# cristicbz/rust-doom

Measured on NVIDIA H100. Metric: frames/sec at 1920x1080 (palette-index bit-exact), higher is better.
Workload: dtype u8

## Files before the change

### rust-doom_b200/csrc/b2d_kernels.cu

```cuda
#include "b2d_kernels.cuh"

namespace b2d {

namespace {

constexpr unsigned kFull = 0xFFFFFFFFu;

constexpr int kMaskWords = 128;
constexpr int kStackDepth = 128;

constexpr uint32_t kVisBit = 1u << 25, kSolidBit = 1u << 24;
__device__ __forceinline__ uint32_t pack_range(int lo, int hi, uint32_t bits) {
    return (uint32_t)lo | ((uint32_t)hi << 12) | bits;
}
__device__ __forceinline__ int range_lo(uint32_t r) { return (int)(r & 0xFFFu); }
__device__ __forceinline__ int range_hi(uint32_t r) { return (int)((r >> 12) & 0xFFFu); }

__device__ __forceinline__ uint32_t word_bits(int w, int lo, int hi) {
    int a = max(lo, w * 32), b = min(hi, w * 32 + 31);
    if (a > b) return 0u;
    uint32_t m = 0xFFFFFFFFu >> (31 - (b - w * 32));
    return m & (0xFFFFFFFFu << (a - w * 32));
}

__device__ __forceinline__ bool range_open(const uint32_t *mask, int lane, int lo, int hi, int passes) {
    bool open = false;
#pragma unroll
    for (int k = 0; k < kMaskWords / 32; k++) {
        if (k >= passes) break;
        int w = lane + 32 * k;
        uint32_t bits = word_bits(w, lo, hi);
        if (bits & ~mask[w]) open = true;
    }
    return __any_sync(kFull, open);
}

__device__ __forceinline__ bool lane_range_open(const uint32_t *mask, int lo, int hi) {
    for (int w = lo >> 5; w <= (hi >> 5); w++)
        if (word_bits(w, lo, hi) & ~mask[w]) return true;
    return false;
}

__device__ __forceinline__ void mark_solid(uint32_t *mask, int lane, int lo, int hi, int passes) {
#pragma unroll
    for (int k = 0; k < kMaskWords / 32; k++) {
        if (k >= passes) break;
        int w = lane + 32 * k;
        uint32_t bits = word_bits(w, lo, hi);
        if (bits) mask[w] |= bits;
    }
}

__host__ __device__ inline size_t align16(size_t v) { return (v + 15) & ~(size_t)15; }

struct WalkSmem {
    size_t off_tx, off_tz, off_segr, off_boxr, off_node, off_ssec, off_sprr, off_sprz, off_mask, off_stack, off_list, total;
};
__host__ __device__ inline WalkSmem walk_layout(int nverts, int nsegs, int nnodes, int nss, int nsprites) {
    WalkSmem L;
    size_t o = 0;
    L.off_tx = o; o = align16(o + 4 * (size_t)nverts);
    L.off_tz = o; o = align16(o + 4 * (size_t)nverts);
    L.off_segr = o; o = align16(o + 4 * (size_t)nsegs);
    L.off_boxr = o; o = align16(o + 8 * (size_t)nnodes);
    L.off_node = o; o = align16(o + 32 * (size_t)nnodes);
    L.off_ssec = o; o = align16(o + 16 * (size_t)nss);
    L.off_sprr = o; o = align16(o + 4 * (size_t)nsprites);
    L.off_sprz = o; o = align16(o + 4 * (size_t)nsprites);
    L.off_mask = o; o = align16(o + 4 * kMaskWords);
    L.off_stack = o; o = align16(o + 4 * kStackDepth);
    L.off_list = o; o = align16(o + 2 * ((size_t)nsegs + (size_t)nsprites));
    L.total = o;
    return L;
}

__device__ __forceinline__ uint32_t smem_addr(const void *p) { return (uint32_t)__cvta_generic_to_shared(p); }
__device__ __forceinline__ void mbar_init(uint64_t *bar, uint32_t arrivals) {
    asm volatile("mbarrier.init.shared::cta.b64 [%0], %1;" ::"r"(smem_addr(bar)), "r"(arrivals));
    asm volatile("fence.mbarrier_init.release.cluster;" ::: "memory");
}
__device__ __forceinline__ void bulk_copy_g2s(void *dst, const void *src, uint32_t bytes, uint64_t *bar) {
    asm volatile("mbarrier.arrive.expect_tx.shared::cta.b64 _, [%0], %1;" ::"r"(smem_addr(bar)), "r"(bytes) : "memory");
    asm volatile("cp.async.bulk.shared::cluster.global.mbarrier::complete_tx::bytes [%0], [%1], %2, [%3];"
                 ::"r"(smem_addr(dst)), "l"(src), "r"(bytes), "r"(smem_addr(bar)) : "memory");
}
__device__ __forceinline__ bool mbar_wait(uint64_t *bar, uint32_t parity) {
    for (int spin = 0; spin < (1 << 24); spin++) {
        uint32_t done;
        asm volatile("{\n\t.reg .pred p;\n\tmbarrier.try_wait.parity.shared::cta.b64 p, [%1], %2;\n\tselp.u32 %0, 1, 0, p;\n\t}"
                     : "=r"(done) : "r"(smem_addr(bar)), "r"(parity) : "memory");
        if (done) return true;
    }
    return false;
}

__global__ void __launch_bounds__(128, 7)
b2d_walk_kernel(const __grid_constant__ DeviceScene sc, const __grid_constant__ View vw, const Pose *__restrict__ poses, int n,
                FrameConst *__restrict__ frames, SegFrame *__restrict__ work, int stride) {
    extern __shared__ __align__(16) uint8_t smem[];
    const int lane = threadIdx.x & 31, warp = threadIdx.x >> 5;
    const int tid = threadIdx.x, nthr = blockDim.x;
    const WalkSmem L = walk_layout(sc.nverts, sc.nsegs, sc.nnodes, sc.nss, sc.nsprites);
    uint8_t *base = smem;
    __shared__ int s_count, s_status;
    __shared__ __align__(8) uint64_t s_bar;
    int32_t *tx = reinterpret_cast<int32_t *>(base + L.off_tx);
    int32_t *tz = reinterpret_cast<int32_t *>(base + L.off_tz);
    uint32_t *segr = reinterpret_cast<uint32_t *>(base + L.off_segr);
    uint32_t *boxr = reinterpret_cast<uint32_t *>(base + L.off_boxr);
    int4 *node_s = reinterpret_cast<int4 *>(base + L.off_node);
    int4 *ssec_s = reinterpret_cast<int4 *>(base + L.off_ssec);
    uint32_t *sprr = reinterpret_cast<uint32_t *>(base + L.off_sprr);
    int32_t *sprz = reinterpret_cast<int32_t *>(base + L.off_sprz);
    uint32_t *mask = reinterpret_cast<uint32_t *>(base + L.off_mask);
    uint32_t *stack = reinterpret_cast<uint32_t *>(base + L.off_stack);
    uint16_t *list = reinterpret_cast<uint16_t *>(base + L.off_list);

    const uint32_t static_bytes = 32u * (uint32_t)sc.nnodes + 16u * (uint32_t)sc.nss;
    bool static_pending = false;
    if (static_bytes) {
        if (tid == 0) mbar_init(&s_bar, 1);
        __syncthreads();
        if (tid == 0) bulk_copy_g2s(node_s, sc.walk_static, static_bytes, &s_bar);
        static_pending = true;
    }
    for (int frame = blockIdx.x; frame < n; frame += gridDim.x) {
    FrameConst fc;
    frame_setup(poses[frame], fc);

    for (int i = tid; i < sc.nverts; i += nthr) {
        int32_t vx = sc.verts[2 * i], vy = sc.verts[2 * i + 1];
        int32_t a, b;
        to_view(fc, vx, vy, a, b);
        tx[i] = a; tz[i] = b;
    }
    __syncthreads();

    for (int i = tid; i < sc.nsegs; i += nthr) {
        const SegRec &S = sc.segs[i];
        uint32_t packed = 0;
        int32_t flags = S.flags;
        if (!(flags & kSegInvalid)) {
            SegFrame sf;
            const bool closes = seg_closes(flags & kSegTwoSided, S.otop, S.obot);
            if (seg_frame_setup(vw, tx[S.v1], tz[S.v1], tx[S.v2], tz[S.v2], sf, closes))
                packed = pack_range(sf.xlo, sf.xhi, kVisBit | (seg_solid(closes, sf) ? kSolidBit : 0u));
        }
        segr[i] = packed;
    }
    for (int i = tid; i < 2 * sc.nnodes; i += nthr) {
        const NodeRec &N = sc.nodes[i >> 1];
        const int32_t *box = (i & 1) ? N.lbox : N.rbox;
        int32_t b4[4] = {box[0], box[1], box[2], box[3]};
        int lo, hi;
        boxr[i] = box_range(fc, vw, b4, lo, hi) ? pack_range(lo, hi, kVisBit) : 0u;
    }
    if (static_pending) {
        if (!mbar_wait(&s_bar, 0)) __trap();
        static_pending = false;
    }
    for (int i = tid; i < sc.nsprites; i += nthr) {
        const SpriteRec &P = sc.sprites[i];
        SpriteFrame sp;
        uint32_t packed = 0;
        sp.cz = 0;
        if (P.tex >= 0 && P.tex < sc.ntex && sprite_setup(fc, vw, P.x, P.y, (int32_t)sc.tex[P.tex].w, sp))
            packed = pack_range(sp.lo, sp.hi, kVisBit);
        sprr[i] = packed;
        sprz[i] = (int32_t)sp.cz;
    }
    for (int w = tid; w < kMaskWords; w += nthr) mask[w] = ~word_bits(w, 0, vw.W - 1);
    if (tid == 0) stack[0] = sc.root;
    __syncthreads();

    const int passes = (vw.W + 1023) / 1024;
    int sp = warp == 0 ? 1 : 0, count = 0, status = 0;
    int budget = 2 * (sc.nnodes + sc.nss) + 64;
    while (sp > 0) {
        if (--budget < 0) { status |= kStatusNoTermination; break; }
        uint32_t child = stack[--sp];
        __syncwarp();
        if (child & kLeaf) {
            uint32_t id = child & 0x7FFFFFFFu;
            if (id >= (uint32_t)sc.nss) continue;
            const int4 ssv = ssec_s[id];
            SSectorRec ss;
            ss.first_seg = ssv.x; ss.num_segs = ssv.y; ss.sector = ssv.z; ss.sprites = ssv.w;
            if (ss.sector < 0) continue;
            {
                const int sfirst = ss.sprites & 0xFFFFFF;
                int scnt = (ss.sprites >> 24) & 0xFF;
                if (sfirst + scnt > sc.nsprites) scnt = sc.nsprites > sfirst ? sc.nsprites - sfirst : 0;
                int nvis = 0;
                for (int k0 = 0; k0 < scnt; k0 += 32) {
                    const int k = k0 + lane, pi = sfirst + k;
                    const uint32_t r = k < scnt ? sprr[pi] : 0u;
                    const bool vis = (r & kVisBit) && lane_range_open(mask, range_lo(r), range_hi(r));
                    int rank = 0, total = 0;
                    const int32_t myz = vis ? sprz[pi] : 0;
                    for (int j0 = 0; j0 < scnt; j0 += 32) {
                        const int j = j0 + lane, pj = sfirst + j;
                        const uint32_t rj = j < scnt ? sprr[pj] : 0u;
                        const bool vj = (rj & kVisBit) && lane_range_open(mask, range_lo(rj), range_hi(rj));
                        const int32_t zj = vj ? sprz[pj] : 0;
                        unsigned mj = __ballot_sync(kFull, vj);
                        total += __popc(mj);
                        while (mj) {
                            const int b = __ffs(mj) - 1;
                            mj &= mj - 1;
                            const int32_t zb = __shfl_sync(kFull, zj, b);
                            const int jb = j0 + b;
                            if (vis && (zb < myz || (zb == myz && jb < k))) rank++;
                        }
                    }
                    const int pos = count + rank;
                    if (vis && pos < sc.nsegs + sc.nsprites) list[pos] = (uint16_t)(sc.nsegs + pi);
                    nvis = total;
                }
                count = min(count + nvis, sc.nsegs + sc.nsprites);
                __syncwarp();
            }
            for (int k0 = 0; k0 < ss.num_segs; k0 += 32) {
                int k = k0 + lane;
                int si = ss.first_seg + k;
                uint32_t r = k < ss.num_segs ? segr[si] : 0u;
                bool vis = (r & kVisBit) && lane_range_open(mask, range_lo(r), range_hi(r));
                unsigned m = __ballot_sync(kFull, vis);
                int pos = count + __popc(m & ((1u << lane) - 1u));
                if (vis && pos < sc.nsegs + sc.nsprites) list[pos] = (uint16_t)si;
                count = min(count + __popc(m), sc.nsegs + sc.nsprites);
                unsigned sm = __ballot_sync(kFull, vis && (r & kSolidBit));
                __syncwarp();
                while (sm) {
                    int j = __ffs(sm) - 1;
                    sm &= sm - 1;
                    uint32_t rj = __shfl_sync(kFull, r, j);
                    mark_solid(mask, lane, range_lo(rj), range_hi(rj), passes);
                }
                __syncwarp();
            }
            if (!range_open(mask, lane, 0, vw.W - 1, passes)) break;
        } else {
            if (child >= (uint32_t)sc.nnodes) continue;
            const int4 nl = node_s[2 * child], nc = node_s[2 * child + 1];
            int side = node_side(fc.pose, nl.x, nl.y, nl.z, nl.w);
            uint32_t near_c = (uint32_t)(side ? nc.y : nc.x), far_c = (uint32_t)(side ? nc.x : nc.y);
            uint32_t rn = boxr[2 * child + side], rf = boxr[2 * child + (side ^ 1)];
            bool far_vis = (rf & kVisBit) && range_open(mask, lane, range_lo(rf), range_hi(rf), passes);
            bool near_vis = (rn & kVisBit) && range_open(mask, lane, range_lo(rn), range_hi(rn), passes);
            int need = (far_vis ? 1 : 0) + (near_vis ? 1 : 0);
            if (sp + need > kStackDepth) { status = kStatusStackOverflow; break; }
            if (lane == 0) {
                int p = sp;
                if (far_vis) stack[p++] = far_c;
                if (near_vis) stack[p++] = near_c;
            }
            sp += need;
            __syncwarp();
        }
    }
    __syncwarp();
    if (warp == 0 && lane == 0) {
        if (count > stride) { count = stride; status |= kStatusWorklistFull; }
        s_count = count; s_status = status;
    }
    __syncthreads();
    count = s_count; status = s_status;

    for (int k = tid; k < count; k += nthr) {
        int si = list[k];
        SegFrame sf;
        if (si >= sc.nsegs) {
            const int pi = si - sc.nsegs;
            const SpriteRec &P = sc.sprites[pi];
            SpriteFrame sp;
            sprite_setup(fc, vw, P.x, P.y, (int32_t)sc.tex[P.tex].w, sp);
            sprite_entry(pi, sp, sf);
            work[(size_t)frame * stride + k] = sf;
            continue;
        }
        const SegRec &S = sc.segs[si];
        seg_frame_setup(vw, tx[S.v1], tz[S.v1], tx[S.v2], tz[S.v2], sf, false);
        sf.seg = si;
        work[(size_t)frame * stride + k] = sf;
    }
    if (tid == 0) {
        if (status) atomicOr(sc.status_flag, status);
        fc.count = count;
        fc.status = status;
#pragma unroll
        for (int i = 0; i < 6; i++) fc.pad[i] = 0;
        frames[frame] = fc;
    }
    __syncthreads();
    }
}

__device__ __forceinline__ uint32_t lds_u32(uint32_t a) {
    uint32_t v;
    asm("ld.shared.u32 %0, [%1];" : "=r"(v) : "r"(a));
    return v;
}

struct RasterCtx {
    const DeviceScene *sc;
    uint32_t pal_s;
    uint2 *rowz;
    PlaneDir dir;
    uint8_t *fb;
    uint32_t *rgba;
    int W, H, x, lane;
    uint32_t skycol;
};

template <bool kRgba>
__device__ __forceinline__ void put_px(const RasterCtx &c, uint8_t *p8, uint32_t *p32, bool on, uint32_t v) {
    if (on) {
        if (kRgba) {
            *p8 = (uint8_t)v;
            *p32 = lds_u32(c.pal_s + 4u * v);
        } else {
            __stcs(p8, (uint8_t)v);
        }
    }
}

__host__ __device__ __forceinline__ bool tex_interleaved(const TexRec &T) { return b2d::tex_interleaved(T.h, T.texel_off); }

constexpr int kBatch = 8;

template <bool kRgba, int kW>
__device__ __forceinline__ void store_batch(const RasterCtx &c, uint8_t *p8, uint32_t *p32, const uint32_t (&v)[kBatch],
                                            int y, int ya, int yb, bool full) {
    const int Wc = kW ? kW : c.W;
    if (full) {
#pragma unroll
        for (int k = 0; k < kBatch; k++) put_px<kRgba>(c, p8 + (size_t)k * Wc, kRgba ? p32 + (size_t)k * Wc : nullptr, true, v[k]);
    } else {
        const uint32_t m = row_mask(y, ya, yb, kBatch);
#pragma unroll
        for (int k = 0; k < kBatch; k++)
            put_px<kRgba>(c, p8 + (size_t)k * Wc, kRgba ? p32 + (size_t)k * Wc : nullptr, (m >> k) & 1u, v[k]);
    }
}

template <bool kRgba, int kW>
__device__ __forceinline__ void fill_void_warp(const RasterCtx &c, int ya, int yb) {
    bool act = ya < yb;
    int y0 = __reduce_min_sync(kFull, act ? ya : 0x7FFFFFFF);
    int y1 = __reduce_max_sync(kFull, act ? yb : 0);
    if (y0 >= y1) return;
    const int Wc = kW ? kW : c.W;
    uint8_t *p8 = c.fb + (size_t)y0 * Wc;
    uint32_t *p32 = kRgba ? c.rgba + (size_t)y0 * Wc : nullptr;
#pragma unroll 1
    for (int y = y0; y < y1; y++, p8 += Wc, p32 += Wc) put_px<kRgba>(c, p8, p32, y >= ya && y < yb, 0u);
}

template <bool kRgba, int kW>
__device__ __forceinline__ void draw_sky_warp(const RasterCtx &c, int ya, int yb) {
    const DeviceScene &sc = *c.sc;
    if (sc.sky_tex < 0) { fill_void_warp<kRgba, kW>(c, ya, yb); return; }
    const TexRec T = sc.tex[sc.sky_tex];
    const bool inter = tex_interleaved(T);
    const uint8_t *px = sc.lit_texels + T.texel_off + (inter ? 4u * c.skycol : c.skycol);
    const uint32_t w4 = 4u * T.w;
    bool act = ya < yb;
    int y0 = __reduce_min_sync(kFull, act ? ya : 0x7FFFFFFF);
    int y1 = __reduce_max_sync(kFull, act ? yb : 0);
    if (y0 >= y1) return;
    const int Wc = kW ? kW : c.W;
    uint8_t *p8 = c.fb + (size_t)y0 * Wc;
    uint32_t *p32 = kRgba ? c.rgba + (size_t)y0 * Wc : nullptr;
#pragma unroll 2
    for (int y = y0; y < y1; y++, p8 += Wc, p32 += Wc) {
        const uint32_t r = sc.skyrow[y];
        put_px<kRgba>(c, p8, p32, y >= ya && y < yb, __ldg(px + (inter ? (r >> 2) * w4 + (r & 3u) : r * T.w)));
    }
}

template <bool kRgba, int kW>
__device__ __forceinline__ void draw_plane_warp(const RasterCtx &c, const FrameConst &fc, const View &vw,
                                                int ya, int yb, int32_t h, int32_t flat, int lightb,
                                                bool visible) {
    const DeviceScene &sc = *c.sc;
    if (!__any_sync(kFull, ya < yb)) return;
    if (!visible) { fill_void_warp<kRgba, kW>(c, ya, yb); return; }
    if (flat == kFlatSky) { draw_sky_warp<kRgba, kW>(c, ya, yb); return; }
    if (flat < 0 || flat >= sc.nflats) { fill_void_warp<kRgba, kW>(c, ya, yb); return; }
    const uint64_t px_hi = reinterpret_cast<uint64_t>(sc.lit_flats) & 0xFFFFFFFF00000000ull;
    const uint32_t habs = plane_habs(h, fc.pose.z);
    bool act = ya < yb;
    int y0 = __reduce_min_sync(kFull, act ? ya : 0x7FFFFFFF);
    int y1 = __reduce_max_sync(kFull, act ? yb : 0);
    const int full_lo = __reduce_max_sync(kFull, act ? ya : 0x7FFFFFFF);
    const int full_hi = __reduce_min_sync(kFull, act ? yb : 0);
    const int Wc = kW ? kW : c.W;
    uint8_t *p8 = c.fb + (size_t)y0 * Wc;
    uint32_t *p32 = kRgba ? c.rgba + (size_t)y0 * Wc : nullptr;
    const uint32_t bu = (uint32_t)fc.pose.x << 10, bv = (uint32_t)fc.pose.y << 10;
    const uint32_t ax = (uint32_t)c.dir.ax, ay = (uint32_t)c.dir.ay;
    for (int yc = y0; yc < y1; yc += 32) {
        int yy = yc + c.lane;
        if (yy < y1) {
            const PlaneRow pr = plane_row(habs, sc.yslope[yy]);
            c.rowz[c.lane] = make_uint2(pr.z8q, (sc.lit_flat_stride >> 6) * (uint32_t)light_row(lightb, pr.z8) + 64u * (uint32_t)flat);
        }
        __syncwarp();
        const int rows = min(32, y1 - yc);
        int j = 0;
        for (; j + kBatch <= rows; j += kBatch, p8 += (size_t)kBatch * Wc, p32 += (size_t)kBatch * Wc) {
            uint32_t v[kBatch];
#pragma unroll
            for (int k = 0; k < kBatch; k++) {
                const uint2 rz = c.rowz[j + k];
                v[k] = __ldg(reinterpret_cast<const uint8_t *>(px_hi | flat_offset(rz.y, bu + rz.x * ax, bv + rz.x * ay)));
            }
            const int y = yc + j;
            store_batch<kRgba, kW>(c, p8, p32, v, y, ya, yb, y >= full_lo && y + kBatch <= full_hi);
        }
        for (; j < rows; j++, p8 += Wc, p32 += Wc) {
            const uint2 rz = c.rowz[j];
            const int y = yc + j;
            put_px<kRgba>(c, p8, p32, y >= ya && y < yb,
                          __ldg(reinterpret_cast<const uint8_t *>(px_hi | flat_offset(rz.y, bu + rz.x * ax, bv + rz.x * ay))));
        }
        __syncwarp();
    }
}

template <bool kRgba, int kW, int R>
__device__ __forceinline__ void wall_fast_loop(const RasterCtx &c, const uint8_t *plq, uint32_t w4, uint32_t nq, uint32_t q,
                                               uint32_t acc, uint32_t ts29, int y0, int y1, int ya, int yb,
                                               int full_lo, int full_hi) {
    const int Wc = kW ? kW : c.W;
    uint8_t *p8 = c.fb + (size_t)y0 * Wc;
    uint32_t *p32 = kRgba ? c.rgba + (size_t)y0 * Wc : nullptr;
    asm("" : "+l"(plq));
#pragma unroll 1
    for (int y = y0; y < y1; y += R, p8 += (size_t)R * Wc, p32 += (size_t)R * Wc) {
        const uint32_t q1 = q + 1u == nq ? 0u : q + 1u;
        const uint32_t w0 = __ldg(reinterpret_cast<const uint32_t *>(plq + (size_t)q * w4));
        const uint32_t w1 = __ldg(reinterpret_cast<const uint32_t *>(plq + (size_t)q1 * w4));
        if (y >= full_lo && y + R <= full_hi) {
#pragma unroll
            for (int k = 0; k < R; k++) {
                uint32_t v = pick_byte(w0, w1, wall_sel(acc, ts29, (uint32_t)k));
                if (kRgba) v &= 0xFFu;
                put_px<kRgba>(c, p8 + (size_t)k * Wc, kRgba ? p32 + (size_t)k * Wc : nullptr, true, v);
            }
        } else {
            const uint32_t m = row_mask(y, ya, yb, R);
#pragma unroll
            for (int k = 0; k < R; k++) {
                uint32_t v = pick_byte(w0, w1, wall_sel(acc, ts29, (uint32_t)k));
                if (kRgba) v &= 0xFFu;
                put_px<kRgba>(c, p8 + (size_t)k * Wc, kRgba ? p32 + (size_t)k * Wc : nullptr, (m >> k) & 1u, v);
            }
        }
        wall_advance(acc, q, ts29, (uint32_t)R, nq);
    }
}

template <bool kRgba, int kW>
__device__ __forceinline__ void draw_wall_warp(const RasterCtx &c, const FrameConst &fc, int ya, int yb,
                                               int32_t tex, int32_t tA, int32_t hA, int32_t ucol,
                                               int32_t iscale, int row) {
    const DeviceScene &sc = *c.sc;
    if (!__any_sync(kFull, ya < yb)) return;
    if (tex < 0 || tex >= sc.ntex) { fill_void_warp<kRgba, kW>(c, ya, yb); return; }
    const TexRec T = sc.tex[tex];
    bool act = ya < yb;
    const uint32_t col = (uint32_t)floormod32(ucol, (int32_t)T.w);
    const uint8_t *pl = sc.lit_texels + (size_t)row * sc.lit_texel_stride + T.texel_off;
    const uint32_t tstep = (uint32_t)(iscale >> 4);
    int y0 = __reduce_min_sync(kFull, act ? ya : 0x7FFFFFFF);
    int y1 = __reduce_max_sync(kFull, act ? yb : 0);
    const int full_lo = __reduce_max_sync(kFull, act ? ya : 0x7FFFFFFF);
    const int full_hi = __reduce_min_sync(kFull, act ? yb : 0);
    uint32_t t = (uint32_t)wall_tbase(tA, hA, fc.pose.z, c.H, iscale) + (uint32_t)y0 * tstep;
    const int Wc = kW ? kW : c.W;
    uint8_t *p8 = c.fb + (size_t)y0 * Wc;
    uint32_t *p32 = kRgba ? c.rgba + (size_t)y0 * Wc : nullptr;
    if (tex_interleaved(T) && T.h >= 8u) {
        const uint32_t ts = act ? tstep : 0u;
        const bool f16 = __all_sync(kFull, ts <= kWallFast16);
        if (f16 || __all_sync(kFull, ts <= kWallFast8)) {
            const uint32_t tt = act ? t : 0u;
            const uint32_t r0 = wall_row((int32_t)tt, T.h, T.hmagic, T.hbias);
            const uint8_t *plq = pl + 4u * col;
            if (f16) wall_fast_loop<kRgba, kW, 16>(c, plq, 4u * T.w, T.h >> 2, r0 >> 2, wall_acc29(tt, r0), ts << 13, y0, y1, ya, yb, full_lo, full_hi);
            else wall_fast_loop<kRgba, kW, 8>(c, plq, 4u * T.w, T.h >> 2, r0 >> 2, wall_acc29(tt, r0), ts << 13, y0, y1, ya, yb, full_lo, full_hi);
            return;
        }
    }
    if (tex_interleaved(T)) {
        const uint32_t colb = 4u * col, w4 = 4u * T.w;
        for (int y = y0; y < y1; y += kBatch, p8 += (size_t)kBatch * Wc, p32 += (size_t)kBatch * Wc, t += (uint32_t)kBatch * tstep) {
            const uint32_t r0 = wall_row((int32_t)t, T.h, T.hmagic, T.hbias);
            const uint32_t acc = wall_acc(t, r0);
            const uint32_t b7 = (acc + 7u * tstep) >> 16;
            uint32_t v[kBatch];
            if (__all_sync(kFull, b7 < 8u)) {
                const uint32_t q0 = r0 >> 2, q1 = next_quad(q0, T.h);
                const uint32_t w0 = __ldg(reinterpret_cast<const uint32_t *>(pl + (q0 * w4 + colb)));
                const uint32_t w1 = __ldg(reinterpret_cast<const uint32_t *>(pl + (q1 * w4 + colb)));
#pragma unroll
                for (int k = 0; k < kBatch; k++) {
                    v[k] = pick_byte(w0, w1, (acc + (uint32_t)k * tstep) >> 16);
                    if (kRgba) v[k] &= 0xFFu;
                }
            } else {
                const uint32_t t4 = t + 4u * tstep;
                const uint32_t r4 = wall_row((int32_t)t4, T.h, T.hmagic, T.hbias);
                const uint32_t acc4 = wall_acc(t4, r4);
                if (__all_sync(kFull, ((acc + 3u * tstep) >> 16) < 8u && ((acc4 + 3u * tstep) >> 16) < 8u)) {
                    const uint32_t q0 = r0 >> 2, q4 = r4 >> 2;
                    const uint32_t a0 = __ldg(reinterpret_cast<const uint32_t *>(pl + (q0 * w4 + colb)));
                    const uint32_t a1 = __ldg(reinterpret_cast<const uint32_t *>(pl + (next_quad(q0, T.h) * w4 + colb)));
                    const uint32_t b0 = __ldg(reinterpret_cast<const uint32_t *>(pl + (q4 * w4 + colb)));
                    const uint32_t b1 = __ldg(reinterpret_cast<const uint32_t *>(pl + (next_quad(q4, T.h) * w4 + colb)));
#pragma unroll
                    for (int k = 0; k < 4; k++) {
                        v[k] = pick_byte(a0, a1, (acc + (uint32_t)k * tstep) >> 16);
                        v[k + 4] = pick_byte(b0, b1, (acc4 + (uint32_t)k * tstep) >> 16);
                        if (kRgba) { v[k] &= 0xFFu; v[k + 4] &= 0xFFu; }
                    }
                } else {
#pragma unroll
                    for (int k = 0; k < kBatch; k++) {
                        const uint32_t rk = wall_row((int32_t)(t + (uint32_t)k * tstep), T.h, T.hmagic, T.hbias);
                        v[k] = __ldg(pl + ((rk >> 2) * w4 + colb + (rk & 3u)));
                    }
                }
            }
            store_batch<kRgba, kW>(c, p8, p32, v, y, ya, yb, y >= full_lo && y + kBatch <= full_hi);
        }
    } else {
        const uint8_t *px = pl + col;
#pragma unroll 1
        for (int y = y0; y < y1; y++, p8 += Wc, p32 += Wc, t += tstep)
            put_px<kRgba>(c, p8, p32, y >= ya && y < yb, __ldg(px + wall_row((int32_t)t, T.h, T.hmagic, T.hbias) * T.w));
    }
}

__device__ __forceinline__ uint32_t *masked_entry(const DeviceScene &sc, const uint32_t *chunks, int e) {
    return sc.masked_list + ((size_t)chunks[e / kMaskedChunk] * kMaskedChunk + (size_t)(e % kMaskedChunk)) * 33u;
}
__device__ __forceinline__ uint32_t *masked_push(const DeviceScene &sc, uint32_t *chunks, int &mcount, int lane) {
    bool ok = mcount < sc.masked_cap;
    if (ok && mcount % kMaskedChunk == 0) {
        uint32_t id = 0;
        if (lane == 0) id = atomicAdd(sc.masked_counter, 1u);
        id = __shfl_sync(kFull, id, 0);
        ok = id < sc.masked_chunks;
        if (ok && lane == 0) chunks[mcount / kMaskedChunk] = id;
        __syncwarp();
    }
    if (!ok) {
        if (lane == 0) atomicOr(sc.status_flag, kStatusMaskedFull);
        return nullptr;
    }
    return masked_entry(sc, chunks, mcount++);
}

template <bool kRgba, int kW>
__device__ __noinline__ void masked_pass(const DeviceScene &sc, const View &vw, int32_t pose_z, uint8_t *fb,
                                         uint32_t *rgba, uint32_t pal_s, int x, int lane,
                                         const SegFrame *wl, const uint32_t *chunks, int count) {
    RasterCtx c;
    c.sc = &sc; c.pal_s = pal_s; c.fb = fb; c.rgba = rgba;
    c.W = vw.W; c.H = vw.H; c.x = x; c.lane = lane;
    const int Wc = kW ? kW : c.W;
    for (int e = count - 1; e >= 0; e--) {
        const uint32_t *ml = masked_entry(sc, chunks, e);
        const uint32_t k = ml[0];
        const uint32_t packed = ml[1 + c.lane];
        int ya = (int)(packed & 0xFFFFu), yb = (int)(packed >> 16);
        const SegFrame sf = wl[k];
        int32_t tex, tA, hA, ucol = 0, iscale = 1, row = 0;
        if (is_sprite_entry(sf)) {
            SpriteFrame sp;
            const SpriteRec P = sc.sprites[entry_sprite(sf, sp)];
            if (P.tex < 0 || P.tex >= sc.ntex) continue;
            const int32_t sw = (int32_t)sc.tex[P.tex].w, sh = (int32_t)sc.tex[P.tex].h;
            const int64_t scale = sprite_scale(vw, sp.cz);
            int32_t z8;
            scale_depth(vw, scale, iscale, z8);
            row = light_row_sprite(P.light, z8);
            tex = P.tex; tA = 0; hA = P.low + sh;
            if (ya < yb) {
                clip_rows(P.low + sh, P.low, (int32_t)scale, pose_z, c.H, ya, yb);
                ucol = sprite_column(sp, vw, c.x, sw);
            }
        } else {
            const SegRec S = sc.segs[sf.seg];
            if (S.mid < 0 || S.mid >= sc.nmids) continue;
            const MidRec M = sc.mids[S.mid];
            tex = M.tex; tA = M.t_high; hA = M.high;
            ColumnEval ce = {0u, 1, 1, 0};
            if (ya < yb && column_eval(sf, vw, c.x, ce)) {
                clip_rows(M.high, M.low, ce.scale, pose_z, c.H, ya, yb);
                ucol = wall_column(S.uoff, S.len_q12, ce.s24);
                iscale = ce.iscale;
                row = light_row(S.light, ce.z8);
            } else {
                ya = yb = 0;
            }
        }
        if (tex < 0 || tex >= sc.ntex) continue;
        const TexRec T = sc.tex[tex];
        const bool act = ya < yb;
        int y0 = __reduce_min_sync(kFull, act ? ya : 0x7FFFFFFF);
        int y1 = __reduce_max_sync(kFull, act ? yb : 0);
        if (y0 >= y1) continue;
        const uint32_t col = (uint32_t)floormod32(ucol, (int32_t)T.w);
        const bool inter = tex_interleaved(T);
        const bool has_mask = T.mask_off != 0xFFFFFFFFu;
        const uint8_t *pl = sc.lit_texels + (size_t)row * sc.lit_texel_stride + T.texel_off;
        const uint8_t *pm = sc.lit_texels + (size_t)32 * sc.lit_texel_stride + T.texel_off;
        const uint32_t tstep = (uint32_t)(iscale >> 4);
        uint32_t t = (uint32_t)wall_tbase(tA, hA, pose_z, c.H, iscale) + (uint32_t)y0 * tstep;
        uint8_t *p8 = c.fb + (size_t)y0 * Wc;
        uint32_t *p32 = kRgba ? c.rgba + (size_t)y0 * Wc : nullptr;
        const uint32_t len = act ? (uint32_t)(yb - ya) : 0u;
        if (inter) {
            const uint32_t colb = 4u * col, w4 = 4u * T.w;
#pragma unroll 1
            for (int y = y0; y < y1; y += kBatch, p8 += (size_t)kBatch * Wc, p32 += (size_t)kBatch * Wc, t += (uint32_t)kBatch * tstep) {
                const uint32_t r0 = wall_row((int32_t)t, T.h, T.hmagic, T.hbias);
                const uint32_t acc = wall_acc(t, r0);
                const uint32_t d = (uint32_t)(y - ya);
                uint32_t v[kBatch], o[kBatch];
                if (__all_sync(kFull, ((acc + 7u * tstep) >> 16) < 8u)) {
                    const uint32_t o0 = (r0 >> 2) * w4 + colb, o1 = next_quad(r0 >> 2, T.h) * w4 + colb;
                    const uint32_t w0 = __ldg(reinterpret_cast<const uint32_t *>(pl + o0));
                    const uint32_t w1 = __ldg(reinterpret_cast<const uint32_t *>(pl + o1));
                    uint32_t m0 = 0x01010101u, m1 = 0x01010101u;
                    if (has_mask) {
                        m0 = __ldg(reinterpret_cast<const uint32_t *>(pm + o0));
                        m1 = __ldg(reinterpret_cast<const uint32_t *>(pm + o1));
                    }
#pragma unroll
                    for (int k = 0; k < kBatch; k++) {
                        const uint32_t bk = (acc + (uint32_t)k * tstep) >> 16;
                        v[k] = pick_byte(w0, w1, bk) & 0xFFu;
                        o[k] = pick_byte(m0, m1, bk) & 0xFFu;
                    }
                } else {
#pragma unroll
                    for (int k = 0; k < kBatch; k++) {
                        const uint32_t rk = wall_row((int32_t)(t + (uint32_t)k * tstep), T.h, T.hmagic, T.hbias);
                        const uint32_t off = (rk >> 2) * w4 + colb + (rk & 3u);
                        v[k] = __ldg(pl + off);
                        o[k] = has_mask ? (uint32_t)__ldg(pm + off) : 1u;
                    }
                }
#pragma unroll
                for (int k = 0; k < kBatch; k++)
                    put_px<kRgba>(c, p8 + (size_t)k * Wc, kRgba ? p32 + (size_t)k * Wc : nullptr, d + (uint32_t)k < len && o[k] != 0u, v[k]);
            }
        } else {
#pragma unroll 1
            for (int y = y0; y < y1; y++, p8 += Wc, p32 += Wc, t += tstep) {
                const uint32_t off = wall_row((int32_t)t, T.h, T.hmagic, T.hbias) * T.w + col;
                const bool on = (uint32_t)(y - ya) < len && (!has_mask || __ldg(pm + off) != 0);
                put_px<kRgba>(c, p8, p32, on, __ldg(pl + off));
            }
        }
    }
}

constexpr int kRasterWarps = 4;

template <bool kRgba, int kW, bool kMasked>
__global__ void __launch_bounds__(32 * kRasterWarps, 16 / kRasterWarps)
b2d_raster_kernel(const __grid_constant__ DeviceScene sc, const __grid_constant__ View vw, const FrameConst *__restrict__ frames,
                  const SegFrame *__restrict__ work, int stride, int n, int strips,
                  uint8_t *__restrict__ index_fb, uint32_t *__restrict__ rgba_fb) {
    __shared__ uint32_t s_pal[kRgba ? 256 : 1];
    __shared__ uint2 s_rowz[kRasterWarps][32];
    __shared__ uint32_t s_chunks[kRasterWarps][kMasked ? kMaskedCapMax / kMaskedChunk : 1];
    if (kRgba) {
        for (int i = threadIdx.x; i < 256; i += blockDim.x) s_pal[i] = sc.palette[i];
        __syncthreads();
    }

    const int lane = threadIdx.x & 31;
    const long long gw = (long long)blockIdx.x * (blockDim.x >> 5) + (threadIdx.x >> 5);
    if (gw >= (long long)n * strips) return;
    const int frame = (int)(gw / strips), strip = (int)(gw % strips);
    const int W = kW ? kW : vw.W, H = vw.H;
    const int x0 = strip * 32, x = x0 + lane;
    const bool inside = x < W;

    const FrameConst fc = frames[frame];
    RasterCtx c;
    c.sc = &sc;
    c.pal_s = (uint32_t)__cvta_generic_to_shared(s_pal);
    c.rowz = s_rowz[threadIdx.x >> 5];
    c.dir = plane_dir(fc, vw, inside ? x : 0, sc.invF);
    c.fb = index_fb + (size_t)frame * W * H + (inside ? x : 0);
    c.rgba = kRgba ? rgba_fb + (size_t)frame * W * H + (inside ? x : 0) : nullptr;
    c.W = W; c.H = H; c.x = x; c.lane = lane;
    c.skycol = 0;
    if (sc.sky_tex >= 0 && inside) c.skycol = umulhi32(sky_u32(x, vw, fc.pose.angle), sc.tex[sc.sky_tex].w);

    int ct = 0, cb = inside ? H : 0;
    uint32_t *chunks = s_chunks[threadIdx.x >> 5];
    asm("" : "+l"(chunks));
    const bool defer = kMasked && sc.masked_list != nullptr;
    int mcount = 0;
    const SegFrame *wl = work + (size_t)frame * stride;
    const int count = fc.count;
    bool done = false;

    for (int k0 = 0; k0 < count && !done; k0 += 32) {
        int k = k0 + lane;
        bool overlap = false;
        if (k < count) {
            int xlo = wl[k].xlo, xhi = wl[k].xhi;
            overlap = xhi >= x0 && xlo <= x0 + 31;
        }
        unsigned m = __ballot_sync(kFull, overlap);
        while (m) {
            int j = __ffs(m) - 1;
            m &= m - 1;
            if (!__any_sync(kFull, ct < cb)) { done = true; break; }
            const SegFrame sf = wl[k0 + j];
            bool in = inside && ct < cb && x >= sf.xlo && x <= sf.xhi;
            if (!__any_sync(kFull, in)) continue;
            if (is_sprite_entry(sf)) {
                if (defer) {
                    uint32_t *ml = masked_push(sc, chunks, mcount, lane);
                    if (ml) {
                        if (lane == 0) ml[0] = (uint32_t)(k0 + j);
                        ml[1 + lane] = in ? ((uint32_t)ct | ((uint32_t)cb << 16)) : 0u;
                    }
                }
                continue;
            }
            ColumnEval ce = {0u, 1, 1, 0};
            bool ok = in && column_eval(sf, vw, x, ce);
            if (!__any_sync(kFull, ok)) continue;

            const SegRec S = sc.segs[sf.seg];
            const SectorRec SF = sc.sectors[S.front];
            const int32_t fcl = SF.ceil, ffl = SF.floor;
            const bool two = S.flags & kSegTwoSided;
            const bool ceil_vis = plane_visible(true, fcl, SF.ceil_flat == kFlatSky, fc.pose.z);
            const bool floor_vis = plane_visible(false, ffl, SF.floor_flat == kFlatSky, fc.pose.z);

            WallRows wr = {ct, ct, ct, ct};
            int yend = ct, row = 0;
            int32_t ucol = 0;
            if (ok) {
                row = light_row(S.light, ce.z8);
                ucol = wall_column(S.uoff, S.len_q12, ce.s24);
                wr = wall_rows(fcl, ffl, two, S.otop, S.obot, ce.scale, fc.pose.z, H, ct, cb);
                yend = cb;
            }
#pragma unroll 1
            for (int pz = 0; pz < 2; pz++) {
                const bool top = pz == 0;
                draw_plane_warp<kRgba, kW>(c, fc, vw, ok ? (top ? ct : wr.y4) : 0, ok ? (top ? wr.y1 : yend) : 0,
                                                    top ? fcl : ffl, top ? SF.ceil_flat : SF.floor_flat, SF.light,
                                                    top ? ceil_vis : floor_vis);
            }
#pragma unroll 1
            for (int pw = 0; pw < 2; pw++) {
                const bool upper = pw == 0;
                if (!wall_piece(upper, two, fcl, ffl, S.otop, S.obot)) continue;
                draw_wall_warp<kRgba, kW>(c, fc, ok ? (upper ? wr.y1 : wr.y3) : 0, ok ? (upper ? wr.y2 : wr.y4) : 0,
                                                   upper ? S.texA : S.texB, upper ? S.tA : S.tB, upper ? S.hA : S.hB,
                                                   ucol, ce.iscale, row);
            }
            if (ok) wall_window(two, wr, H, ct, cb);
            if (defer && two && S.mid >= 0) {
                const bool keep = ok && wr.y2 < wr.y3;
                if (__any_sync(kFull, keep)) {
                    uint32_t *ml = masked_push(sc, chunks, mcount, lane);
                    if (ml) {
                        if (lane == 0) ml[0] = (uint32_t)(k0 + j);
                        ml[1 + lane] = keep ? ((uint32_t)wr.y2 | ((uint32_t)wr.y3 << 16)) : 0u;
                    }
                }
            }
        }
    }
    fill_void_warp<kRgba, kW>(c, inside ? ct : 0, inside ? cb : 0);
    if (kMasked && mcount > 0) {
        __syncwarp();
        masked_pass<kRgba, kW>(sc, vw, fc.pose.z, c.fb, c.rgba, c.pal_s, x, lane, wl, chunks, mcount);
    }
}

__global__ void __launch_bounds__(256)
b2d_palette_kernel(const uint32_t *__restrict__ palette, const uint8_t *__restrict__ index,
                   uint32_t *__restrict__ rgba, size_t n_pixels) {
    __shared__ uint32_t s_pal[256];
    s_pal[threadIdx.x] = palette[threadIdx.x];
    __syncthreads();
    const bool aligned = ((reinterpret_cast<uintptr_t>(index) | reinterpret_cast<uintptr_t>(rgba)) & 15) == 0;
    const size_t nvec = aligned ? n_pixels / 16 : 0;
    const size_t stride = (size_t)gridDim.x * blockDim.x;
    for (size_t i = (size_t)blockIdx.x * blockDim.x + threadIdx.x; i < nvec; i += stride) {
        uint4 in = __ldcs(reinterpret_cast<const uint4 *>(index) + i);
        uint32_t wds[4] = {in.x, in.y, in.z, in.w};
        uint4 *out = reinterpret_cast<uint4 *>(rgba) + 4 * i;
#pragma unroll
        for (int q = 0; q < 4; q++) {
            uint4 o;
            o.x = s_pal[wds[q] & 0xFF];
            o.y = s_pal[(wds[q] >> 8) & 0xFF];
            o.z = s_pal[(wds[q] >> 16) & 0xFF];
            o.w = s_pal[wds[q] >> 24];
            __stcs(out + q, o);
        }
    }
    for (size_t p = nvec * 16 + (size_t)blockIdx.x * blockDim.x + threadIdx.x; p < n_pixels; p += stride)
        rgba[p] = s_pal[index[p]];
}

}

size_t walk_smem_per_warp(const DeviceScene &sc) { return walk_layout(sc.nverts, sc.nsegs, sc.nnodes, sc.nss, sc.nsprites).total; }

static int device_sms() {
    int dev = 0, sms = 0;
    cudaGetDevice(&dev);
    cudaDeviceGetAttribute(&sms, cudaDevAttrMultiProcessorCount, dev);
    return sms > 0 ? sms : 1;
}

cudaError_t launch_walk(const DeviceScene &sc, const View &vw, const Pose *d_poses, int n,
                        FrameConst *d_frames, SegFrame *d_work, int stride, cudaStream_t stream, bool background) {
    if (n <= 0) return cudaSuccess;
    const size_t smem = walk_smem_per_warp(sc);
    if (smem > 227 * 1024) return cudaErrorInvalidValue;
    if (smem > 48 * 1024) {
        cudaError_t e = cudaFuncSetAttribute(b2d_walk_kernel, cudaFuncAttributeMaxDynamicSharedMemorySize, (int)smem);
        if (e != cudaSuccess) return e;
    }
    const int sms = device_sms();
    const int blocks = (background && n > sms) ? sms : n, warps = 4;
    b2d_walk_kernel<<<blocks, warps * 32, smem, stream>>>(sc, vw, d_poses, n, d_frames, d_work, stride);
    return cudaGetLastError();
}

cudaError_t launch_raster(const DeviceScene &sc, const View &vw, const FrameConst *d_frames,
                          const SegFrame *d_work, int stride, int n, uint8_t *d_index_fb,
                          uint32_t *d_rgba, cudaStream_t stream) {
    if (n <= 0) return cudaSuccess;
    const int strips = (vw.W + 31) / 32;
    const int nblocks = (int)(((long long)n * strips + kRasterWarps - 1) / kRasterWarps);
    const bool masked = (sc.nmids > 0 || sc.nsprites > 0) && sc.masked_list;
#define B2D_RASTER_GO(RGBA, KW) do { \
    if (masked) b2d_raster_kernel<RGBA, KW, true><<<nblocks, 32 * kRasterWarps, 0, stream>>>(sc, vw, d_frames, d_work, stride, n, strips, d_index_fb, d_rgba); \
    else b2d_raster_kernel<RGBA, KW, false><<<nblocks, 32 * kRasterWarps, 0, stream>>>(sc, vw, d_frames, d_work, stride, n, strips, d_index_fb, d_rgba); \
    } while (0)
    if (d_rgba) { if (vw.W == 1920) B2D_RASTER_GO(true, 1920); else B2D_RASTER_GO(true, 0); }
    else if (vw.W == 1920) B2D_RASTER_GO(false, 1920);
    else if (vw.W == 3840) B2D_RASTER_GO(false, 3840);
    else B2D_RASTER_GO(false, 0);
#undef B2D_RASTER_GO
    return cudaGetLastError();
}

namespace {
__global__ void __launch_bounds__(256)
b2d_prelight_kernel(const uint8_t *__restrict__ colormap, const uint8_t *__restrict__ src, uint8_t *__restrict__ dst,
                    size_t n, size_t stride) {
    __shared__ uint8_t cm[32 * 256];
    for (int i = threadIdx.x; i < 32 * 256; i += blockDim.x) cm[i] = colormap[i];
    __syncthreads();
    for (size_t i = (size_t)blockIdx.x * blockDim.x + threadIdx.x; i < n; i += (size_t)gridDim.x * blockDim.x) {
        const uint32_t t = src[i];
#pragma unroll 4
        for (int r = 0; r < 32; r++) dst[(size_t)r * stride + i] = cm[r * 256 + t];
    }
}
}

namespace {
__global__ void __launch_bounds__(256)
b2d_prelight_tex_kernel(const uint8_t *__restrict__ colormap, const uint8_t *__restrict__ texels,
                        const TexRec *__restrict__ tex, int ntex, uint8_t *__restrict__ dst, size_t stride) {
    __shared__ uint8_t cm[32 * 256];
    for (int i = threadIdx.x; i < 32 * 256; i += blockDim.x) cm[i] = colormap[i];
    __syncthreads();
    for (int ti = blockIdx.x; ti < ntex; ti += gridDim.x) {
        const TexRec T = tex[ti];
        const bool inter = tex_interleaved(T);
        const uint32_t n = T.w * T.h;
        for (uint32_t i = threadIdx.x; i < n; i += blockDim.x) {
            const uint32_t row = i / T.w, col = i - row * T.w;
            const uint32_t o = lit_index(inter, T.w, row, col);
            const uint32_t t = texels[T.texel_off + i];
            for (int r = 0; r < 32; r++) dst[(size_t)r * stride + T.texel_off + o] = cm[r * 256 + t];
            if (T.mask_off != 0xFFFFFFFFu) dst[(size_t)32 * stride + T.texel_off + o] = texels[T.mask_off + i];
        }
    }
}
}

cudaError_t launch_prelight_textures(const uint8_t *d_colormap, const uint8_t *d_texels, const TexRec *d_tex, int ntex,
                                     uint8_t *d_dst, size_t stride, cudaStream_t stream) {
    if (ntex <= 0) return cudaSuccess;
    const int cap = device_sms() * 8;
    b2d_prelight_tex_kernel<<<ntex < cap ? ntex : cap, 256, 0, stream>>>(d_colormap, d_texels, d_tex, ntex, d_dst, stride);
    return cudaGetLastError();
}

cudaError_t launch_prelight(const uint8_t *d_colormap, const uint8_t *d_src, uint8_t *d_dst, size_t n, size_t stride,
                            cudaStream_t stream) {
    if (n == 0) return cudaSuccess;
    int blocks = (int)((n + 255) / 256);
    if (blocks > device_sms() * 8) blocks = device_sms() * 8;
    b2d_prelight_kernel<<<blocks, 256, 0, stream>>>(d_colormap, d_src, d_dst, n, stride);
    return cudaGetLastError();
}

cudaError_t launch_palette(const uint32_t *d_palette, const uint8_t *d_index, uint32_t *d_rgba,
                           size_t n_pixels, cudaStream_t stream) {
    if (n_pixels == 0) return cudaSuccess;
    size_t nvec = n_pixels / 16 + 1;
    int blocks = (int)((nvec + 255) / 256);
    const int cap = device_sms() * 16;
    if (blocks > cap) blocks = cap;
    b2d_palette_kernel<<<blocks, 256, 0, stream>>>(d_palette, d_index, d_rgba, n_pixels);
    return cudaGetLastError();
}

}
```

Baseline: 507,600.

## Process raster segments in lockstep across block warps for unmasked scenes

Maps each block to a 128-column group of one frame. In the unmasked variant all four warps walk the union of segments overlapping the group and check early termination with a block-wide __syncthreads_and, so warps of one block advance together through the same segment records. The intent is better cache sharing of segment, sector and texture data across neighbouring strips. In exchange, warps that have already closed wait on the slowest warp and pay a block barrier on every segment step.

```diff
diff --git a/rust-doom_b200/csrc/b2d_kernels.cu b/rust-doom_b200/csrc/b2d_kernels.cu
--- a/rust-doom_b200/csrc/b2d_kernels.cu
+++ b/rust-doom_b200/csrc/b2d_kernels.cu
@@ -672,11 +672,12 @@
 }
 
 constexpr int kRasterWarps = 4;
+constexpr int kGroupCols = 32 * kRasterWarps;
 
 template <bool kRgba, int kW, bool kMasked>
 __global__ void __launch_bounds__(32 * kRasterWarps, 16 / kRasterWarps)
 b2d_raster_kernel(const __grid_constant__ DeviceScene sc, const __grid_constant__ View vw, const FrameConst *__restrict__ frames,
-                  const SegFrame *__restrict__ work, int stride, int n, int strips,
+                  const SegFrame *__restrict__ work, int stride, int groups,
                   uint8_t *__restrict__ index_fb, uint32_t *__restrict__ rgba_fb) {
     __shared__ uint32_t s_pal[kRgba ? 256 : 1];
     __shared__ uint2 s_rowz[kRasterWarps][32];
@@ -687,11 +688,10 @@
     }
 
     const int lane = threadIdx.x & 31;
-    const long long gw = (long long)blockIdx.x * (blockDim.x >> 5) + (threadIdx.x >> 5);
-    if (gw >= (long long)n * strips) return;
-    const int frame = (int)(gw / strips), strip = (int)(gw % strips);
+    const int frame = (int)(blockIdx.x / (unsigned)groups), group = (int)(blockIdx.x % (unsigned)groups);
     const int W = kW ? kW : vw.W, H = vw.H;
-    const int x0 = strip * 32, x = x0 + lane;
+    const int g0 = group * kGroupCols;
+    const int x0 = g0 + 32 * (threadIdx.x >> 5), x = x0 + lane;
     const bool inside = x < W;
 
     const FrameConst fc = frames[frame];
@@ -715,77 +715,84 @@
     const int count = fc.count;
     bool done = false;
 
+    constexpr bool kUnison = !kMasked;
     for (int k0 = 0; k0 < count && !done; k0 += 32) {
         int k = k0 + lane;
-        bool overlap = false;
+        bool in_group = false, in_strip = false;
         if (k < count) {
             int xlo = wl[k].xlo, xhi = wl[k].xhi;
-            overlap = xhi >= x0 && xlo <= x0 + 31;
-        }
-        unsigned m = __ballot_sync(kFull, overlap);
+            in_group = xhi >= g0 && xlo <= g0 + kGroupCols - 1;
+            in_strip = xhi >= x0 && xlo <= x0 + 31;
+        }
+        const unsigned mine = __ballot_sync(kFull, in_strip);
+        unsigned m = kUnison ? __ballot_sync(kFull, in_group) : mine;
         while (m) {
             int j = __ffs(m) - 1;
             m &= m - 1;
-            if (!__any_sync(kFull, ct < cb)) { done = true; break; }
-            const SegFrame sf = wl[k0 + j];
-            bool in = inside && ct < cb && x >= sf.xlo && x <= sf.xhi;
-            if (!__any_sync(kFull, in)) continue;
-            if (is_sprite_entry(sf)) {
-                if (defer) {
-                    uint32_t *ml = masked_push(sc, chunks, mcount, lane);
-                    if (ml) {
-                        if (lane == 0) ml[0] = (uint32_t)(k0 + j);
-                        ml[1 + lane] = in ? ((uint32_t)ct | ((uint32_t)cb << 16)) : 0u;
+            do {
+                if (!((mine >> j) & 1u)) break;
+                const SegFrame sf = wl[k0 + j];
+                bool in = inside && ct < cb && x >= sf.xlo && x <= sf.xhi;
+                if (!__any_sync(kFull, in)) break;
+                if (is_sprite_entry(sf)) {
+                    if (defer) {
+                        uint32_t *ml = masked_push(sc, chunks, mcount, lane);
+                        if (ml) {
+                            if (lane == 0) ml[0] = (uint32_t)(k0 + j);
+                            ml[1 + lane] = in ? ((uint32_t)ct | ((uint32_t)cb << 16)) : 0u;
+                        }
+                    }
+                    break;
+                }
+                ColumnEval ce = {0u, 1, 1, 0};
+                bool ok = in && column_eval(sf, vw, x, ce);
+                if (!__any_sync(kFull, ok)) break;
+
+                const SegRec S = sc.segs[sf.seg];
+                const SectorRec SF = sc.sectors[S.front];
+                const int32_t fcl = SF.ceil, ffl = SF.floor;
+                const bool two = S.flags & kSegTwoSided;
+                const bool ceil_vis = plane_visible(true, fcl, SF.ceil_flat == kFlatSky, fc.pose.z);
+                const bool floor_vis = plane_visible(false, ffl, SF.floor_flat == kFlatSky, fc.pose.z);
+
+                WallRows wr = {ct, ct, ct, ct};
+                int yend = ct, row = 0;
+                int32_t ucol = 0;
+                if (ok) {
+                    row = light_row(S.light, ce.z8);
+                    ucol = wall_column(S.uoff, S.len_q12, ce.s24);
+                    wr = wall_rows(fcl, ffl, two, S.otop, S.obot, ce.scale, fc.pose.z, H, ct, cb);
+                    yend = cb;
+                }
+#pragma unroll 1
+                for (int pz = 0; pz < 2; pz++) {
+                    const bool top = pz == 0;
+                    draw_plane_warp<kRgba, kW>(c, fc, vw, ok ? (top ? ct : wr.y4) : 0, ok ? (top ? wr.y1 : yend) : 0,
+                                                        top ? fcl : ffl, top ? SF.ceil_flat : SF.floor_flat, SF.light,
+                                                        top ? ceil_vis : floor_vis);
+                }
+#pragma unroll 1
+                for (int pw = 0; pw < 2; pw++) {
+                    const bool upper = pw == 0;
+                    if (!wall_piece(upper, two, fcl, ffl, S.otop, S.obot)) continue;
+                    draw_wall_warp<kRgba, kW>(c, fc, ok ? (upper ? wr.y1 : wr.y3) : 0, ok ? (upper ? wr.y2 : wr.y4) : 0,
+                                                       upper ? S.texA : S.texB, upper ? S.tA : S.tB, upper ? S.hA : S.hB,
+                                                       ucol, ce.iscale, row);
+                }
+                if (ok) wall_window(two, wr, H, ct, cb);
+                if (defer && two && S.mid >= 0) {
+                    const bool keep = ok && wr.y2 < wr.y3;
+                    if (__any_sync(kFull, keep)) {
+                        uint32_t *ml = masked_push(sc, chunks, mcount, lane);
+                        if (ml) {
+                            if (lane == 0) ml[0] = (uint32_t)(k0 + j);
+                            ml[1 + lane] = keep ? ((uint32_t)wr.y2 | ((uint32_t)wr.y3 << 16)) : 0u;
+                        }
                     }
                 }
-                continue;
-            }
-            ColumnEval ce = {0u, 1, 1, 0};
-            bool ok = in && column_eval(sf, vw, x, ce);
-            if (!__any_sync(kFull, ok)) continue;
-
-            const SegRec S = sc.segs[sf.seg];
-            const SectorRec SF = sc.sectors[S.front];
-            const int32_t fcl = SF.ceil, ffl = SF.floor;
-            const bool two = S.flags & kSegTwoSided;
-            const bool ceil_vis = plane_visible(true, fcl, SF.ceil_flat == kFlatSky, fc.pose.z);
-            const bool floor_vis = plane_visible(false, ffl, SF.floor_flat == kFlatSky, fc.pose.z);
-
-            WallRows wr = {ct, ct, ct, ct};
-            int yend = ct, row = 0;
-            int32_t ucol = 0;
-            if (ok) {
-                row = light_row(S.light, ce.z8);
-                ucol = wall_column(S.uoff, S.len_q12, ce.s24);
-                wr = wall_rows(fcl, ffl, two, S.otop, S.obot, ce.scale, fc.pose.z, H, ct, cb);
-                yend = cb;
-            }
-#pragma unroll 1
-            for (int pz = 0; pz < 2; pz++) {
-                const bool top = pz == 0;
-                draw_plane_warp<kRgba, kW>(c, fc, vw, ok ? (top ? ct : wr.y4) : 0, ok ? (top ? wr.y1 : yend) : 0,
-                                                    top ? fcl : ffl, top ? SF.ceil_flat : SF.floor_flat, SF.light,
-                                                    top ? ceil_vis : floor_vis);
-            }
-#pragma unroll 1
-            for (int pw = 0; pw < 2; pw++) {
-                const bool upper = pw == 0;
-                if (!wall_piece(upper, two, fcl, ffl, S.otop, S.obot)) continue;
-                draw_wall_warp<kRgba, kW>(c, fc, ok ? (upper ? wr.y1 : wr.y3) : 0, ok ? (upper ? wr.y2 : wr.y4) : 0,
-                                                   upper ? S.texA : S.texB, upper ? S.tA : S.tB, upper ? S.hA : S.hB,
-                                                   ucol, ce.iscale, row);
-            }
-            if (ok) wall_window(two, wr, H, ct, cb);
-            if (defer && two && S.mid >= 0) {
-                const bool keep = ok && wr.y2 < wr.y3;
-                if (__any_sync(kFull, keep)) {
-                    uint32_t *ml = masked_push(sc, chunks, mcount, lane);
-                    if (ml) {
-                        if (lane == 0) ml[0] = (uint32_t)(k0 + j);
-                        ml[1 + lane] = keep ? ((uint32_t)wr.y2 | ((uint32_t)wr.y3 << 16)) : 0u;
-                    }
-                }
-            }
+            } while (false);
+            const bool closed = !__any_sync(kFull, ct < cb);
+            if (kUnison ? __syncthreads_and(closed) : closed) { done = true; break; }
         }
     }
     fill_void_warp<kRgba, kW>(c, inside ? ct : 0, inside ? cb : 0);
@@ -852,12 +859,12 @@
                           const SegFrame *d_work, int stride, int n, uint8_t *d_index_fb,
                           uint32_t *d_rgba, cudaStream_t stream) {
     if (n <= 0) return cudaSuccess;
-    const int strips = (vw.W + 31) / 32;
-    const int nblocks = (int)(((long long)n * strips + kRasterWarps - 1) / kRasterWarps);
+    const int groups = (vw.W + kGroupCols - 1) / kGroupCols;
+    const int nblocks = n * groups;
     const bool masked = (sc.nmids > 0 || sc.nsprites > 0) && sc.masked_list;
 #define B2D_RASTER_GO(RGBA, KW) do { \
-    if (masked) b2d_raster_kernel<RGBA, KW, true><<<nblocks, 32 * kRasterWarps, 0, stream>>>(sc, vw, d_frames, d_work, stride, n, strips, d_index_fb, d_rgba); \
-    else b2d_raster_kernel<RGBA, KW, false><<<nblocks, 32 * kRasterWarps, 0, stream>>>(sc, vw, d_frames, d_work, stride, n, strips, d_index_fb, d_rgba); \
+    if (masked) b2d_raster_kernel<RGBA, KW, true><<<nblocks, 32 * kRasterWarps, 0, stream>>>(sc, vw, d_frames, d_work, stride, groups, d_index_fb, d_rgba); \
+    else b2d_raster_kernel<RGBA, KW, false><<<nblocks, 32 * kRasterWarps, 0, stream>>>(sc, vw, d_frames, d_work, stride, groups, d_index_fb, d_rgba); \
     } while (0)
     if (d_rgba) { if (vw.W == 1920) B2D_RASTER_GO(true, 1920); else B2D_RASTER_GO(true, 0); }
     else if (vw.W == 1920) B2D_RASTER_GO(false, 1920);
```

Result: faster. 522,200 (median of 6 runs) (+2.9%).
